# MeshFEM/MeshFEM

Measured on AMD Instinct MI355X. Metric: stiffness_assembly_elements_per_s, higher is better.
Workload: dtype f64; 1 GPU; configs[2]: 60^3 grid -> 5184000 P2 tets, isotropic E=200 nu=0.35, Dirichlet x=0, traction x=1; elements=5184000, nodes=7430761, dof=22292283, nnz_blocks=201443041, stored_blocks=104436901, matrix_storage=upper, parallelism=1 GPU, step=embed + Ke blocks + assembly into block-CSR (gather/owner-computes)

## Files before the change

meshfem_amd/csrc/mfh_api.cpp:

```cpp
#include "mfh_ctx.hh"
#include <dlfcn.h>

using namespace mfh;

namespace {
struct RoctxApi {
    int (*push)(const char *) = nullptr;
    int (*pop)() = nullptr;
    RoctxApi() {
        const char *en = getenv("MFH_ROCTX");
        if (!en || en[0] == '0') return;
        for (const char *lib : {"librocprofiler-sdk-roctx.so", "libroctx64.so", "/opt/rocm/lib/librocprofiler-sdk-roctx.so", "/opt/rocm/lib/libroctx64.so"}) {
            if (void *h = dlopen(lib, RTLD_NOW | RTLD_GLOBAL)) {
                push = reinterpret_cast<int (*)(const char *)>(dlsym(h, "roctxRangePushA"));
                pop = reinterpret_cast<int (*)()>(dlsym(h, "roctxRangePop"));
                if (push && pop) return;
                push = nullptr; pop = nullptr;
            }
        }
    }
};
RoctxApi &roctx_api() { static RoctxApi a; return a; }
}
mfh::RoctxRange::RoctxRange(const char *name) {
// ... 44 lines not shown
    c->neumannTraction.assign((size_t)m.nBE() * m.dim, 0.0);
    const size_t n = m.bdryNodes.size() * (size_t)m.dim;
    if (n > 0 && c->dirMask.size() == n && c->dirVal.size() == n) {
        parallel_assign(c->dirMask, n, (uint8_t)0);
        parallel_assign(c->dirVal, n, 0.0);
    } else {
        RawVec<uint8_t>().swap(c->dirMask);
        RawVec<double>().swap(c->dirVal);
    }
    c->deltaForces.clear();
}
void clear_fixed(mfh_ctx *c) {
    c->fixedVars.clear();
    c->fixedVals.clear();
    if (c->hFixedMask.size() == (size_t)c->bs() * c->nDoF) parallel_assign(c->hFixedMask, c->hFixedMask.size(), (uint8_t)0);
    else RawVec<uint8_t>().swap(c->hFixedMask);
    c->fixedUploaded = false;
    c->anyFixedNonzero = false;
    c->dinvValid = false;
    c->tl.valid = false;
    c->mg.valid = false;
}

void upload_mesh(mfh_ctx *c, bool deviceTables) {
    double t0 = now_ms();
    c->autoStretch = -1.0;
    if (!c->hostOnly && !deviceTables) {
        require_device(c);
        MFH_HIP(hipSetDevice(c->device));
        c->dElemNodes.upload(c->mesh.elemNodes, c->stream);
        c->dVertPos.upload(c->mesh.nodePos, c->stream);
    }
    c->timing.upload_ms = now_ms() - t0;
    c->haveMesh = true;
    c->external = false;
    c->geoValid = false;
    c->hGeoValid = false;
    c->dofForNode.clear();
    c->nDoF = c->mesh.nNode;
    build_shape_tables(c->mesh.dim, c->mesh.deg, c->tables);
    if (!c->hostOnly) { c->dPairTable.upload(c->tables.pairTable, c->stream); c->dMassTable.upload(c->tables.massRef, c->stream); }
    invalidate_symbolic(c);
    dist_detach(c);
    reset_bcs(c);
    clear_fixed(c);
}

void set_isotropic(mfh_ctx *c, double E, double nu) {
    double lam = (nu * E) / ((1.0 + nu) * (1.0 - 2.0 * nu));
    if (c->haveMesh && c->mesh.dim == 2) lam = (nu * E) / (1.0 - nu * nu);
    c->matMode = 0;
    c->matKind = MAT_ISO;
    c->matParams = {lam, E / (2.0 + 2.0 * nu), E, nu};
    c->geoValid = false;
    c->hGeoValid = false;
    invalidate_matrix(c);
}

void ensure_pass_events(mfh_ctx *c) {
    if (c->passEv[0]) return;
    for (auto &e : c->passEv) MFH_HIP(hipEventCreate(&e));
    MFH_HIP(hipHostMalloc((void **)&c->negHost, 2 * sizeof(int), hipHostMallocDefault));
}

void ensure_geometry(mfh_ctx *c, bool deferCheck) {
    require(c->haveMesh, MFH_ERR_STATE, "no mesh set");
    if (c->geoValid) return;
    require(!c->hostOnly, MFH_ERR_HIP, "host-only context (device -1): no HIP device, and there is no CPU fallback");
    require_device(c);
    MFH_HIP(hipSetDevice(c->device));
    const HostMesh &m = c->mesh;
    if (c->matParams.empty() && !c->dMatBorrowed) set_isotropic(c, 1.0, 0.3);
    if (c->matMode == 0 && !c->dMatBorrowed) {
        double E = c->matParams[2], nu = c->matParams[3];
        double lam = (nu * E) / ((1.0 + nu) * (1.0 - 2.0 * nu));
        if (m.dim == 2) lam = (nu * E) / (1.0 - nu * nu);
        c->matParams[0] = lam;
    }
    c->geoStride = c->matKind == MAT_ISO ? GEO_ISO_STRIDE : (c->matKind == MAT_ORTHO ? GEO_ORTHO_STRIDE : GEO_GEN_STRIDE);
    if (!c->dMatBorrowed) c->dMatParams.upload(c->matParams, c->stream);
    const double *dMat = c->dMatBorrowed ? c->dMatBorrowed : c->dMatParams.p;
    c->dGeo.alloc((size_t)m.nElem * c->geoStride);
    c->dNeg.alloc(2);
    c->dNeg.zero(c->stream);
    ensure_pass_events(c);
    MFH_HIP(hipEventRecord(c->passEv[0], c->stream));
    k::launch_geometry(m.dim, m.deg, c->matKind, m.nElem, c->dElemNodes.p, m.npe, c->dVertPos.p, dMat, c->matMode,
                       c->dGeo.p, c->geoStride, c->dNeg.p, c->stream);
    MFH_HIP(hipEventRecord(c->passEv[1], c->stream));
    MFH_HIP(hipMemcpyAsync(c->negHost, c->dNeg.p, 2 * sizeof(int), hipMemcpyDeviceToHost, c->stream));
    c->geoPending = true;
    if (!deferCheck) finish_geometry(c);
}

void finish_geometry(mfh_ctx *c) {
    if (!c->geoPending) return;
    c->geoPending = false;
    MFH_HIP(hipStreamSynchronize(c->stream));
    float ms = 0;
    MFH_HIP(hipEventElapsedTime(&ms, c->passEv[0], c->passEv[1]));
    c->timing.geometry_ms = ms;
    const int neg[2] = {c->negHost[0], c->negHost[1]};
    if (neg[0] > 0)
        throw Error(MFH_ERR_INVALID, "Mesh has negatively oriented elements.\nCorrect with: mesh_convert --reorientNegativeElements. (" +
                                         std::to_string(neg[0]) + " elements)");
    if (neg[1] > 0)
        throw Error(MFH_ERR_INVALID, std::string(c->matMode == 1 ? "Isotropic" : "Orthotropic") + " parameters of " + std::to_string(neg[1]) +
                                         " elements give an indefinite elasticity tensor (" +
                                         (c->matMode == 1 ? "need E > 0 and -1 < nu < 1/2, nu < 1 in plane stress" : "compliance matrix not positive definite") + ").");
    c->geoValid = true;
    c->hGeoValid = false;
}

const std::vector<double> &host_geo(mfh_ctx *c) {
    ensure_geometry(c);
    if (!c->hGeoValid) {
        c->hGeo.resize(c->dGeo.n);
        c->dGeo.download(c->hGeo.data(), c->dGeo.n, c->stream);
        c->hGeoValid = true;
    }
    return c->hGeo;
}

const int32_t *device_dof_map(mfh_ctx *c) {
    if (c->dofForNode.empty()) return nullptr;
    if (!c->dofUploaded) { c->dDofForNode.upload(c->dofForNode, c->stream); c->dofUploaded = true; }
    return c->dDofForNode.p;
}

void ensure_host_colidx(mfh_ctx *c) {
    if (!c->sym.colIdx.empty() || c->sym.nnzb == 0) return;
    c->sym.colIdx.resize((size_t)c->sym.nnzb);
    c->dColIdx.download(c->sym.colIdx.data(), c->sym.colIdx.size(), c->stream);
}

void refresh_storage_rule(mfh_ctx *c) {
    if (c->symValid && resolve_upper_storage(c) != c->upperOnly) { c->symValid = false; invalidate_matrix(c); }
}

void ensure_symbolic(mfh_ctx *c, bool wantScatter) {
    require(c->haveMesh, MFH_ERR_STATE, "no mesh set");
    refresh_storage_rule(c);
    if (c->symValid && (!wantScatter || c->symHasScatter)) return;
    c->upperOnly = resolve_upper_storage(c);
    RoctxRange range("Compress Matrix");
    double t0 = now_ms();
    if (!c->hostOnly && c->symbolicDevice && c->contribOrder == 1) {
        require_device(c);
        MFH_HIP(hipSetDevice(c->device));
        const bool directPacked = c->asmPackedCodes && !c->keepHostSymbolic;
// ... 27 lines not shown
        invalidate_matrix(c);
        return;
    }
    build_symbolic(c->mesh, c->dofForNode, c->nDoF, c->nOwnedDoF(), c->chunkSlots, c->contribOrder, wantScatter, c->sym, c->upperOnly);
    c->timing.symbolic_ms = now_ms() - t0;
    const Symbolic &S = c->sym;
    c->symHasScatter = wantScatter;
    if (c->hostOnly) { c->symValid = true; return; }
    MFH_HIP(hipSetDevice(c->device));
    c->dRowPtr.upload(S.rowPtr, c->stream);
    c->dColIdx.upload(S.colIdx, c->stream);
    c->dChunkRow.upload(S.chunkRow, c->stream);
    c->dSpmvChunkRow.upload(S.spmvChunkRow, c->stream);
    c->dContribPtr.upload(S.contribPtr, c->stream);
    c->dContribCode.upload(S.contribCode, c->stream);
    c->dContribSlot.upload(S.contribSlot, c->stream);
    if (wantScatter) c->dScatter.upload(S.scatterSlot, c->stream);
    pack_gather_codes(c);
    if (!c->keepHostSymbolic) {
        std::vector<uint32_t>().swap(c->sym.contribCode);
        std::vector<uint16_t>().swap(c->sym.contribSlot);
        std::vector<int32_t>().swap(c->sym.scatterSlot);
    }
    { mfh::PoolTag values(c->hierarchyLevel ? 0 : 1); c->dVals.alloc(tiled_count(S.nnzb, c->dim() * c->dim())); }
    c->symValid = true;
    ++c->listsGen;
    ++c->valsGen;
    invalidate_matrix(c);
}

void pack_gather_codes(mfh_ctx *c) {
    c->codesPacked = false;
    if (!c->asmPackedCodes || c->hostOnly || c->sym.nChunk() == 0) return;
    c->dChunkElemBase.alloc((size_t)c->sym.nChunk());
    DBuf<int> flag;
    flag.alloc(1);
    c->codesPacked = k::launch_pack_codes(c->sym.nChunk(), c->dContribPtr.p, c->dContribCode.p, c->mesh.npe, c->dChunkElemBase.p, flag.p, c->stream);
}

k::AsmArgs asm_args(mfh_ctx *c) {
    const HostMesh &m = c->mesh;
    k::AsmArgs a{};
    a.dim = m.dim; a.deg = m.deg; a.npe = m.npe; a.mat = c->asmMat();
    a.geoStride = c->geoStride; a.geo = c->dGeo.p; a.pairTable = c->dPairTable.p; a.massTable = c->dMassTable.p;
    for (int k2 = 0; k2 < 6; ++k2) a.pairConst[k2] = c->tables.pairConst[k2];
    a.nChunk = c->sym.nChunk(); a.chunkRow = c->dChunkRow.p; a.rowPtr = c->dRowPtr.p;
    a.contribPtr = c->dContribPtr.p; a.contribCode = c->dContribCode.p; a.contribSlot = c->dContribSlot.p;
    a.chunkSlots = c->sym.chunkSlots;
    a.nElem = m.nElem; a.scatterSlot = c->dScatter.p;
    a.vals = c->dVals.p; a.nnzb = c->sym.nnzb;
    a.xcd = c->xcdSwizzle;
    a.upperOnly = c->upperOnly ? 1 : 0;
    a.det = c->deterministic ? 1 : 0;
    a.chunkElemBase = c->codesPacked ? c->dChunkElemBase.p : nullptr;
    a.chunkOrder = nullptr;
    if (c->asmChunkOrder && !c->hostOnly && a.nChunk > 1 && c->symValid && c->dContribPtr.p && c->dContribCode.p && c->contribOrder == 1) {
        if (c->chunkOrderGen != c->listsGen) {
            DBuf<uint32_t> keys;
            keys.alloc((size_t)a.nChunk);
            k::launch_chunk_keys(a, keys.p, c->stream);
            std::vector<uint32_t> hk((size_t)a.nChunk);
            keys.download(hk.data(), hk.size(), c->stream);
            std::vector<int32_t> order((size_t)a.nChunk);
            for (int64_t b = 0; b < a.nChunk; ++b) order[(size_t)b] = (int32_t)b;
            std::stable_sort(order.begin(), order.end(), [&](int32_t x, int32_t y) { return hk[(size_t)x] < hk[(size_t)y]; });
            c->dChunkOrder.upload(order, c->stream);
            c->chunkOrderGen = c->listsGen;
        }
        a.chunkOrder = c->dChunkOrder.p;
    }
    return a;
}

void run_assembly(mfh_ctx *c, int mode) {
    c->dVals32.release();
    k::AsmArgs a = asm_args(c);
    if (mode == MFH_ASSEMBLE_ATOMIC) {
        c->dVals.zero(c->stream);
        k::launch_assemble_atomic(a, c->stream);
    } else {
        k::launch_assemble_gather(a, c->stream);
    }
}

void placement_trials(mfh_ctx *c) {
    c->placementGen = c->valsGen;
    c->placementMs.clear();
    c->placementNote.clear();
    const size_t n = c->dVals.n, bytes = n * sizeof(double);
    if (c->placementTrials <= 0 || c->hostOnly || c->external || bytes < ((size_t)256 << 20)) return;
    auto timed = [&]() {
        k::AsmArgs a = asm_args(c);
        double best = 1e300;
        for (int r = 0; r < 2; ++r) {
            EventTimer t(c->stream);
            k::launch_assemble_gather(a, c->stream);
            best = std::min(best, t.stop());
        }
        return best;
    };
    double best = timed();
    c->placementMs.push_back(best);
    std::vector<std::unique_ptr<DBuf<double>>> held;
    for (int trial = 0; trial < c->placementTrials; ++trial) {
        size_t fr = 0, tot = 0;
        if (hipMemGetInfo(&fr, &tot) != hipSuccess) { (void)hipGetLastError(); break; }
// ... 810 lines not shown
    std::copy(c->mesh.bdryParent.begin(), c->mesh.bdryParent.end(), out);
    return MFH_OK;
}
mfh_status mfh_mesh_get_boundary_elem_internal(const mfh_ctx *c, uint8_t *out) {
    if (!c || !c->haveMesh || !out) return MFH_ERR_STATE;
    std::copy(c->mesh.bdryInternal.begin(), c->mesh.bdryInternal.end(), out);
    return MFH_OK;
}
mfh_status mfh_mesh_get_boundary_nodes(const mfh_ctx *c, int32_t *out) {
    if (!c || !c->haveMesh || !out) return MFH_ERR_STATE;
    std::copy(c->mesh.bdryNodes.begin(), c->mesh.bdryNodes.end(), out);
    return MFH_OK;
}
mfh_status mfh_mesh_get_boundary_elem_geometry(const mfh_ctx *c, double *volume, double *normal) {
    if (!c || !c->haveMesh) return MFH_ERR_STATE;
    if (volume) std::copy(c->mesh.bdryVol.begin(), c->mesh.bdryVol.end(), volume);
    if (normal) std::copy(c->mesh.bdryNormal.begin(), c->mesh.bdryNormal.end(), normal);
    return MFH_OK;
}
mfh_status mfh_mesh_get_elem_volumes(mfh_ctx *c, double *out) {
    MFH_TRY(c)
    require(c && out, MFH_ERR_INVALID, "null argument");
    const std::vector<double> &g = host_geo(c);
    for (int64_t e = 0; e < c->mesh.nElem; ++e) out[e] = g[(size_t)e * c->geoStride + 12];
    MFH_CATCH(c)
}

mfh_status mfh_material_isotropic(mfh_ctx *c, double E, double nu) {
    MFH_TRY(c)
    require(c, MFH_ERR_INVALID, "null context");
    set_isotropic(c, E, nu);
    MFH_CATCH(c)
}

mfh_status mfh_material_const(mfh_ctx *c, const double *D) {
    MFH_TRY(c)
    require(c && D && c->haveMesh, MFH_ERR_STATE, "set the mesh before the material");
    const int d = c->dim(), fl = flat_len(d);
    c->matParams.clear();
    bool ortho = true;
    for (int r = 0; r < fl && ortho; ++r)
        for (int cc = r + 1; cc < fl; ++cc)
            if (cc >= d && D[r * fl + cc] != 0.0) { ortho = false; break; }
    if (ortho) {
        for (int r = 0; r < d; ++r)
            for (int cc = r; cc < d; ++cc) c->matParams.push_back(D[r * fl + cc]);
        for (int k2 = d; k2 < fl; ++k2) c->matParams.push_back(D[k2 * fl + k2]);
        c->matMode = 5; c->matKind = MAT_ORTHO;
    } else {
        for (int r = 0; r < fl; ++r)
            for (int cc = r; cc < fl; ++cc) c->matParams.push_back(D[r * fl + cc]);
        c->matMode = 2; c->matKind = MAT_GENERAL;
    }
    c->geoValid = false; c->hGeoValid = false;
    invalidate_matrix(c);
    MFH_CATCH(c)
}

mfh_status mfh_material_iso_field(mfh_ctx *c, const double *E, const double *nu) {
    MFH_TRY(c)
    require(c && E && nu && c->haveMesh, MFH_ERR_STATE, "set the mesh before the material");
    const int64_t n = c->mesh.nElem;
    c->matParams.assign((size_t)2 * n, 0.0);
    std::copy(E, E + n, c->matParams.begin());
    std::copy(nu, nu + n, c->matParams.begin() + n);
    c->matMode = 1; c->matKind = MAT_ISO;
    c->geoValid = false; c->hGeoValid = false;
    invalidate_matrix(c);
    MFH_CATCH(c)
}

mfh_status mfh_material_ortho_field(mfh_ctx *c, const double *params) {
    MFH_TRY(c)
    require(c && params && c->haveMesh, MFH_ERR_STATE, "set the mesh before the material");
    const int np = c->dim() == 3 ? 9 : 4;
    c->matParams.assign(params, params + (size_t)np * c->mesh.nElem);
    c->matMode = 3; c->matKind = MAT_ORTHO;
    c->geoValid = false; c->hGeoValid = false;
    invalidate_matrix(c);
    MFH_CATCH(c)
}

mfh_status mfh_material_tensor_field(mfh_ctx *c, const double *D) {
    MFH_TRY(c)
    require(c && D && c->haveMesh, MFH_ERR_STATE, "set the mesh before the material");
    const int fl = flat_len(c->dim());
    c->matParams.assign(D, D + (size_t)fl * fl * c->mesh.nElem);
    c->matMode = 4; c->matKind = MAT_GENERAL;
    c->geoValid = false; c->hGeoValid = false;
    invalidate_matrix(c);
    MFH_CATCH(c)
}

mfh_status mfh_material_get(mfh_ctx *c, int64_t elem, double *D) {
    MFH_TRY(c)
    require(c && D && c->haveMesh && elem >= 0 && elem < c->mesh.nElem, MFH_ERR_INVALID, "bad element");
    const std::vector<double> &g = host_geo(c);
    elem_D(c, &g[(size_t)elem * c->geoStride], D);
    MFH_CATCH(c)
}

mfh_status mfh_dof_map(mfh_ctx *c, const int32_t *dofForNode, int64_t nDoF) {
    MFH_TRY(c)
    require(c && c->haveMesh, MFH_ERR_STATE, "no mesh set");
    c->nOwnedDoFSet = -1;
    if (!dofForNode) {
        c->dofForNode.clear();
        c->nDoF = c->mesh.nNode;
        std::fill(c->mesh.bdryInternal.begin(), c->mesh.bdryInternal.end(), (uint8_t)0);
    } else {
        require(c->mesh.nOwned == c->mesh.nNode, MFH_ERR_UNSUPPORTED, "a DoF map on a partitioned mesh says which DoFs are this rank's rows: mfh_dof_map_partitioned");
        require(nDoF > 0 && nDoF <= c->mesh.nNode, MFH_ERR_INVALID, "bad nDoF");
        for (int64_t n = 0; n < c->mesh.nNode; ++n)
            require(dofForNode[n] >= 0 && dofForNode[n] < nDoF, MFH_ERR_INVALID, "DoF index out of range");
        c->dofForNode.assign(dofForNode, dofForNode + c->mesh.nNode);
        c->nDoF = nDoF;
    }
    invalidate_symbolic(c);
    clear_fixed(c);
    MFH_CATCH(c)
}

mfh_status mfh_dof_map_partitioned(mfh_ctx *c, const int32_t *dofForNode, int64_t nDoF, int64_t nOwnedDoF) {
    MFH_TRY(c)
    require(c && c->haveMesh && dofForNode, MFH_ERR_STATE, "no mesh set");
    require(!c->mesh.hasTopology, MFH_ERR_UNSUPPORTED, "partitioned contexts are built by mfh_mesh_set");
    require(nDoF > 0 && nDoF <= c->mesh.nNode && nOwnedDoF > 0 && nOwnedDoF <= nDoF, MFH_ERR_INVALID, "bad DoF counts");
    for (int64_t n = 0; n < c->mesh.nNode; ++n)
        require(dofForNode[n] >= 0 && dofForNode[n] < nDoF, MFH_ERR_INVALID, "DoF index out of range");
    c->dofForNode.assign(dofForNode, dofForNode + c->mesh.nNode);
    c->nDoF = nDoF;
    c->nOwnedDoFSet = nOwnedDoF;
    invalidate_symbolic(c);
    clear_fixed(c);
    dist_detach(c);
    MFH_CATCH(c)
}

mfh_status mfh_apply_periodic_conditions(mfh_ctx *c, double eps, int64_t *nDoF) {
    MFH_TRY(c)
    require(c && c->haveMesh, MFH_ERR_STATE, "no mesh set");
// ... 764 lines not shown
```

meshfem_amd/csrc/mfh_ctx.hh:

```
#pragma once
#include "mfh_internal.hh"
#include <cmath>
#include <map>
#include <mutex>

using namespace mfh;

struct mfh_ctx {
    int device = 0;
    bool hostOnly = false;
    bool hierarchyLevel = false;
    bool keepHostSymbolic = false;
    int xcdSwizzle = 0;
    RawVec<double> hLoad, hX, hXBatch, hLoadBatch;
    bool alwaysReembed = false;
    bool deterministic = false;
    DBuf<double> detPartials;
    DBuf<unsigned> detCounter;
    bool periodicIgnoreMismatch = false;
    int periodicIgnoreDims = 0;
    hipStream_t stream = nullptr;
    bool ownStream = true;
    bool arenaCounted = false;
    std::string err;

    HostMesh mesh;
    bool haveMesh = false;
    bool external = false;
    DBuf<int32_t> dElemNodes;
    DBuf<double> dVertPos;

    int matMode = 0;
    int matKind = MAT_ISO;
    int op = MFH_OP_ELASTICITY;
    std::vector<double> matParams;
    DBuf<double> dMatParams;
    const double *dMatBorrowed = nullptr;
    DBuf<double> dGeo;
    DBuf<int> dNeg;
    int geoStride = GEO_ISO_STRIDE;
    bool geoValid = false;
    hipEvent_t passEv[4] = {nullptr, nullptr, nullptr, nullptr};
    int *negHost = nullptr;
    bool geoPending = false;
    std::vector<double> hGeo;
    bool hGeoValid = false;

    std::vector<int32_t> dofForNode;
    DBuf<int32_t> dDofForNode;
    bool dofUploaded = false;
    int64_t nDoF = 0;

    Symbolic sym;
    bool symValid = false;
    bool symHasScatter = false;
    DBuf<int32_t> dRowPtr, dColIdx, dChunkRow, dSpmvChunkRow, dScatter;
    DBuf<int64_t> dContribPtr;
    int matrixStorage = -1;
    bool upperOnly = false;
    int nCU = 256;
    DBuf<uint32_t> dContribCode;
    DBuf<uint16_t> dContribSlot;
    ShapeTables tables;
    DBuf<double> dPairTable, dMassTable;
    MfLists mf;
    bool mfValid = false;
    int matrixFree = -1;
    bool use_mf() const {
        if (external || !haveMesh || hostOnly) return false;
        return matrixFree == 1 || (matrixFree < 0 && op == MFH_OP_ELASTICITY);
    }
    DBuf<int32_t> dMfChunkRow;
    DBuf<int64_t> dMfPairPtr;
    DBuf<uint32_t> dMfPairCode, dMfPairPos;
    DBuf<uint16_t> dMfPairRow;
    MfClusterLists mfc;
    MfClusterDev mfcDev;
    bool mfcValid = false;
    int mfXcdGroup = 32;
    bool mfReorder = true;
    DBuf<int32_t> dMfElemPerm, dMfElemNodes;
    int mfLaneStride = 37;
    bool mfGeoFromVerts = true;
    int mfBlockElems = 0;
    DBuf<double> dMfSig;
    int mfChunkRows = 256, mfChunkPairs = 2048;
    bool mfClusterUnfit = false;
    int mfModeEff() const { return (mfMode == 4 && mfClusterUnfit) ? 3 : mfMode; }
    int mfMode = 4;
// ... 304 lines not shown
```

meshfem_amd/csrc/mfh_internal.hh:

```
#pragma once
#include <hip/hip_runtime.h>
#include <cstdint>
#include <cstdio>
#include <cstring>
#include <string>
#include <vector>
#include <stdexcept>
#include <chrono>
#include <thread>
#include <functional>
#include <algorithm>
#include <array>
#include <memory>
#include <cstdlib>
#include "../../include/meshfem_hip.h"
#include "../../include/meshfem_hip_extras.h"

namespace mfh {

struct Error : std::runtime_error {
    mfh_status code;
    Error(mfh_status c, const std::string &m) : std::runtime_error(m), code(c) {}
};

// ... 267 lines not shown
void build_aggregates_device(int dim, int64_t nDoF, const double *dPos, int targetNodes, hipStream_t s, Aggregates &A,
                             DBuf<int32_t> &dAggOfDof, DBuf<double> &dRelPos, DBuf<int32_t> &dAggPtr, DBuf<int32_t> &dDofsByAgg,
                             const double *globalBox = nullptr, int64_t globalCount = 0, bool fullLattice = false, const double *aspect = nullptr);
void element_extent_sums_device(int dim, int64_t nElem, int npe, const int32_t *dElemNodes, const double *dPos, hipStream_t s, double out[3]);
void bounding_box_device(int dim, int64_t nDoF, const double *dPos, hipStream_t s, double mn[3], double mx[3]);
void wrap_positions_device(int64_t n, int dim, const double box[6], hipStream_t s, double *dPos, int skipDims = 0);
bool spd_inverse_inplace(int64_t n, double *A);
void build_mg_transfer_device(const HostMesh &m, const int32_t *dElemNodes, hipStream_t s, DBuf<int32_t> &parA, DBuf<int32_t> &parB,
                              DBuf<int32_t> &fineOf, DBuf<int32_t> &resPtr, DBuf<int32_t> &resIdx);

}

namespace mfh { namespace k {

struct DetBuf {
    double *partials = nullptr;
    unsigned *counter = nullptr;
    int cap = 0;
};
extern thread_local DetBuf t_det;
struct DetScope {
    DetBuf saved;
    explicit DetScope(const DetBuf &d) : saved(t_det) { t_det = d; }
    ~DetScope() { t_det = saved; }
    DetScope(const DetScope &) = delete;
    DetScope &operator=(const DetScope &) = delete;
};
inline int det_grid(int grid) { return t_det.partials ? std::min(grid, t_det.cap) : grid; }
void launch_det_finish(hipStream_t s);

struct AsmArgs {
    int dim, deg, npe, mat;
    int geoStride;
    const double *geo;
    const double *pairTable;
    const double *massTable;
    double pairConst[6];
    int64_t nChunk;
    const int32_t *chunkRow;
    const int32_t *rowPtr;
    const int64_t *contribPtr;
    const uint32_t *contribCode;
    const uint16_t *contribSlot;
    int chunkSlots;
    int64_t nElem;
    const int32_t *scatterSlot;
    double *vals;
    int64_t nnzb;
    int xcd;
    const int32_t *chunkElemBase;
    const int32_t *chunkOrder;
    int upperOnly;
    int det;
};

void launch_geometry(int dim, int deg, int mat, int64_t nElem, const int32_t *elemNodes, int npe,
                     const double *vertPos, const double *matParams, int matMode, double *geo, int geoStride,
                     int *negCount, hipStream_t s);
void launch_assemble_gather(const AsmArgs &a, hipStream_t s);
void launch_chunk_keys(const AsmArgs &a, uint32_t *keys, hipStream_t s);
bool launch_pack_codes(int64_t nChunk, const int64_t *contribPtr, uint32_t *contribCode, int npe, int32_t *chunkElemBase, int *flag, hipStream_t s);
void launch_assemble_atomic(const AsmArgs &a, hipStream_t s);
void launch_element_stiffness(const AsmArgs &a, int64_t first, int64_t count, double *KeOut, hipStream_t s);
void launch_constant_strain_load(const AsmArgs &a, const int32_t *elemNodes, const int32_t *dofForNode, const double *intGrad,
                                 const double *cstrain, const double *deltaP, double *out, hipStream_t s);
void launch_average_strain(const AsmArgs &a, const int32_t *elemNodes, const double *intGrad, const double *uNodes, double *out,
                           int wantStress, const double *uFixed, const double *deltaP, hipStream_t s, const double *addStrain = nullptr,
                           double *integral = nullptr);
void launch_apply_delta_K(const AsmArgs &a, const int32_t *elemNodes, const int32_t *dofForNode, const double *intGrad,
                          const double *uNodes, const double *deltaP, double *out, hipStream_t s);
void launch_mutual_energies(const AsmArgs &a, const int32_t *elemNodes, const double *intGrad, const double *w, int64_t nNode,
                            const double *deltaP, double *out, hipStream_t s);
void launch_boundary_strain_field(const AsmArgs &a, const int32_t *elemNodes, const double *intGrad, int64_t nBE,
                                  const int32_t *bdryParent, const int32_t *bdryElemNodes, int npbe, const double *uNodes,
                                  int wantStress, double *out, hipStream_t s);
void launch_strain_field(const AsmArgs &a, const int32_t *elemNodes, const double *intGrad, const double *uNodes, int wantStress,
                         double *out, hipStream_t s);
void launch_mutual_energy_differential(const AsmArgs &a, const int32_t *elemNodes, const double *intGrad, const double *w,
                                       int64_t nNode, int64_t nVert, double *out, hipStream_t s);
void launch_average_gradient(const AsmArgs &a, const int32_t *elemNodes, const double *intGrad, const double *uNodes, double *out,
                             hipStream_t s);

struct SpmvArgs {
    int dim;
    int64_t nChunk;
    const int32_t *chunkRow;
    const int32_t *rowPtr;
    const int32_t *colIdx;
    const double *vals;
    const float *vals32;
    int chunkSlots;
    const uint8_t *fixedMask;
    int xcd;
    int pcgMode;
    DetBuf det;
};
struct SpmvMfArgs {
    int dim, deg, npe, mat;
    int64_t nChunk;
    const int32_t *chunkRow;
    const int64_t *pairPtr;
    const uint32_t *pairCode;
    const uint16_t *pairRow;
    const uint32_t *pairPos;
    const int32_t *elemNodes;
    const int32_t *dofForNode;
// ... 154 lines not shown
```

meshfem_amd/csrc/mfh_kernels.hip:

```cpp
#include "mfh_device.hh"

namespace mfh { namespace k {

template <int DIM, int MAT> DEV constexpr int mat_nb() { return (MAT == MAT_LAPLACE || MAT == MAT_MASS) ? 1 : DIM * DIM; }

template <int DIM, int MAT>
DEV void block_from_H(const double *__restrict__ g, const double (&H)[DIM][DIM], double *K);

template <int DIM>
DEV void pair_H(const double *__restrict__ g, uint32_t offs , double S0, double S1, double S2,
                double S3, double (&H)[DIM][DIM]) {
#ifndef MFH_ASM_ABLATE
#define MFH_ASM_ABLATE 0
#endif
    const double vol = MFH_ASM_ABLATE >= 1 ? 1.0 : g[12];
    S0 *= vol; S1 *= vol; S2 *= vol; S3 *= vol;
    const char *gb = reinterpret_cast<const char *>(g);
    const double *gsi = reinterpret_cast<const double *>(gb + (offs & 0xffu)), *gti = reinterpret_cast<const double *>(gb + ((offs >> 8) & 0xffu)),
                 *gsj = reinterpret_cast<const double *>(gb + ((offs >> 16) & 0xffu)), *gtj = reinterpret_cast<const double *>(gb + (offs >> 24));
    double ua[DIM], ub[DIM], p[DIM], q[DIM];
#pragma unroll
    for (int a = 0; a < DIM; ++a) {
        ua[a] = MFH_ASM_ABLATE >= 1 ? S0 + a : gsi[a]; ub[a] = MFH_ASM_ABLATE >= 1 ? S1 - a : gti[a];
        const double va = MFH_ASM_ABLATE >= 2 ? S2 + a : gsj[a], vb = MFH_ASM_ABLATE >= 2 ? S3 - a : gtj[a];
        p[a] = S0 * va + S1 * vb;
        q[a] = S2 * va + S3 * vb;
    }
#pragma unroll
    for (int a = 0; a < DIM; ++a)
#pragma unroll
        for (int b = 0; b < DIM; ++b) H[a][b] = ua[a] * p[b] + ub[a] * q[b];
}

template <int DIM, int DEG, int MAT>
DEV void elem_block(const double *__restrict__ g, const double *__restrict__ pairTab, const PairConst &pc, int i, int j, double *K) {
    constexpr int NPE = (DIM == 3) ? (DEG == 1 ? 4 : 10) : (DEG == 1 ? 3 : 6);
    const double vol = g[12];
    if (MAT == MAT_MASS) {
        K[0] = vol * pairTab[i * NPE + j];
        return;
    }
    double H[DIM][DIM];
    if (DEG == 1) {
        double gi[DIM], gj[DIM];
#pragma unroll
        for (int a = 0; a < DIM; ++a) { gi[a] = g[i * DIM + a]; gj[a] = g[j * DIM + a] * vol; }
#pragma unroll
        for (int a = 0; a < DIM; ++a)
#pragma unroll
            for (int b = 0; b < DIM; ++b) H[a][b] = gi[a] * gj[b];
    } else {
        const int si = sup_s<DIM, DEG>(i), ti = sup_t<DIM, DEG>(i), sj = sup_s<DIM, DEG>(j), tj = sup_t<DIM, DEG>(j);
        constexpr int NV = DIM + 1;
        const bool vi = i < NV, vj = j < NV;
        const int lAi = vi ? si : ti, lBi = si, lAj = vj ? sj : tj, lBj = sj;
        const double c1 = pc.ee_ne, c2 = pc.ee_eq - pc.ee_ne, c3 = pc.ee_ne - pc.ve_ne;
        const double oi = vi ? 1.0 : 0.0, oj = vj ? 1.0 : 0.0;
        auto coef = [&](bool eq, double o, double o2) -> double { return (c1 + (eq ? c2 : 0.0)) - c3 * (o + o2) + o * o2; };
        double S0 = coef(lAi == lAj, oi, oj);
        double S1 = vj ? 0.0 : coef(lAi == lBj, oi, 0.0);
        double S2 = vi ? 0.0 : coef(lBi == lAj, 0.0, oj);
        double S3 = (vi | vj) ? 0.0 : coef(lBi == lBj, 0.0, 0.0);
        S0 *= vol; S1 *= vol; S2 *= vol; S3 *= vol;
        double ua[DIM], ub[DIM], p[DIM], q[DIM];
#pragma unroll
        for (int a = 0; a < DIM; ++a) {
            ua[a] = g[si * DIM + a]; ub[a] = g[ti * DIM + a];
            const double va = g[sj * DIM + a], vb = g[tj * DIM + a];
            p[a] = S0 * va + S1 * vb;
            q[a] = S2 * va + S3 * vb;
        }
#pragma unroll
        for (int a = 0; a < DIM; ++a)
#pragma unroll
            for (int b = 0; b < DIM; ++b) H[a][b] = ua[a] * p[b] + ub[a] * q[b];
    }
    block_from_H<DIM, MAT>(g, H, K);
}

template <int DIM, int MAT>
DEV void block_from_H(const double *__restrict__ g, const double (&H)[DIM][DIM], double *K) {
    if (MAT == MAT_LAPLACE) {
        double tr = 0;
#pragma unroll
        for (int a = 0; a < DIM; ++a) tr += H[a][a];
        K[0] = tr;
    } else if (MAT == MAT_ISO) {
#if defined(MFH_ASM_ABLATE) && MFH_ASM_ABLATE >= 1
        const double lam = H[0][0], mu = H[1][1];
#else
        const double lam = g[13], mu = g[14];
#endif
        double tr = 0;
#pragma unroll
        for (int a = 0; a < DIM; ++a) tr += H[a][a];
#pragma unroll
        for (int c = 0; c < DIM; ++c)
#pragma unroll
            for (int d = 0; d < DIM; ++d) K[c * DIM + d] = lam * H[c][d] + mu * H[d][c] + (c == d ? mu * tr : 0.0);
    } else if (MAT == MAT_ORTHO) {
#pragma unroll
        for (int c = 0; c < DIM; ++c)
#pragma unroll
            for (int d = 0; d < DIM; ++d) {
                double v = g[13 + npack<DIM>(c, d)] * H[c][d];
                if (c == d) {
#pragma unroll
                    for (int a = 0; a < DIM; ++a)
                        if (a != c) v += g[ortho_shear_offset<DIM>() + flat_idx<DIM>(a, c) - DIM] * H[a][a];
                } else v += g[ortho_shear_offset<DIM>() + flat_idx<DIM>(c, d) - DIM] * H[d][c];
                K[c * DIM + d] = v;
            }
    } else {
        constexpr int ND = (DIM * (DIM + 1) / 2) * (DIM * (DIM + 1) / 2 + 1) / 2;
        double D[ND];
#pragma unroll
        for (int k = 0; k < ND; ++k) D[k] = g[13 + k];
#pragma unroll
        for (int c = 0; c < DIM; ++c)
#pragma unroll
            for (int d = 0; d < DIM; ++d) {
                double acc = 0;
#pragma unroll
                for (int a = 0; a < DIM; ++a)
#pragma unroll
                    for (int b = 0; b < DIM; ++b) acc += H[a][b] * D[dpack<DIM>(flat_idx<DIM>(a, c), flat_idx<DIM>(d, b))];
                K[c * DIM + d] = acc;
            }
    }
}

template <int DIM>
DEV void embed_simplex(const double (&P)[DIM + 1][DIM], double (&gl)[DIM + 1][DIM], double &vol) {
    if (DIM == 3) {
        auto cross = [](const double *a, const double *b, double *o) {
            o[0] = a[1] * b[2] - a[2] * b[1]; o[1] = a[2] * b[0] - a[0] * b[2]; o[2] = a[0] * b[1] - a[1] * b[0];
        };
        double d31[3], d21[3], d01[3], d20[3], d30[3], d10[3], n[4][3];
#pragma unroll
        for (int a = 0; a < 3; ++a) {
            d31[a] = P[3][a] - P[1][a]; d21[a] = P[2][a] - P[1][a]; d01[a] = P[0][a] - P[1][a];
            d20[a] = P[2][a] - P[0][a]; d30[a] = P[3][a] - P[0][a]; d10[a] = P[1][a] - P[0][a];
        }
        cross(d31, d21, n[0]); cross(d20, d30, n[1]); cross(d30, d10, n[2]); cross(d10, d20, n[3]);
        const double vol6 = d01[0] * n[0][0] + d01[1] * n[0][1] + d01[2] * n[0][2];
        vol = vol6 / 6.0;
#pragma unroll
        for (int k = 0; k < 4; ++k)
#pragma unroll
            for (int a = 0; a < 3; ++a) gl[k][a] = n[k][a] / vol6;
    } else {
        double E[3][2];
// ... 63 lines not shown
            const double *q = mp + e * 4;
            const double a00 = 1.0 / q[0], a01 = -q[2] / q[1], a11 = 1.0 / q[1];
            const double det = a00 * a11 - a01 * a01;
            if (!(a00 > 0 && det > 0 && q[3] > 0)) atomicAdd(negCount + 1, 1);
            g[13 + npack<2>(0, 0)] = a11 / det; g[13 + npack<2>(0, 1)] = -a01 / det; g[13 + npack<2>(1, 1)] = a00 / det;
            g[ortho_shear_offset<2>()] = q[3];
        }
    } else {
        const double *q = mp + e * FL * FL;
        for (int r = 0; r < FL; ++r)
            for (int c = r; c < FL; ++c) g[13 + dpack<DIM>(r, c)] = q[r * FL + c];
    }
    }
    __syncthreads();
    const int64_t e0 = (int64_t)blockIdx.x * blockDim.x;
    const int nLive = (int)(nElem - e0 < (int64_t)blockDim.x ? nElem - e0 : (int64_t)blockDim.x);
    double *out = geo + e0 * stride;
    for (int q = threadIdx.x; q < nLive * stride; q += blockDim.x) {
        const int el = q / stride;
        out[q] = recs[(size_t)el * (stride + 1) + (q - el * stride)];
    }
}

template <int DIM, int DEG, int MAT> DEV constexpr bool asm_uses_table() { return DEG == 2 && MAT != MAT_MASS; }
constexpr int ASM_CODE_SHIFT = 7;

template <int DIM, int DEG, int MAT, bool UPPER = false, bool DET = false>
__global__ void __launch_bounds__(256, (MAT == MAT_GENERAL || MAT == MAT_ORTHO) ? 1 : 8) k_assemble_gather(AsmArgs a) {
    constexpr int NB = mat_nb<DIM, MAT>();
    constexpr int NPE = (DIM == 3) ? (DEG == 1 ? 4 : 10) : (DEG == 1 ? 3 : 6);
    constexpr bool TAB = asm_uses_table<DIM, DEG, MAT>();
    extern __shared__ __attribute__((aligned(16))) double acc[];
    const int CS = a.chunkSlots + 2;
    double *tabS = acc + (size_t)NB * CS;
    uint32_t *tabO = reinterpret_cast<uint32_t *>(tabS + NPE * NPE * 4);
    uint32_t *turn = tabO + NPE * NPE;
    const PairConst pc{a.pairConst[0], a.pairConst[1], a.pairConst[2], a.pairConst[3], a.pairConst[4], a.pairConst[5]};
    const int64_t item = a.xcd == 1 ? xcd_item(blockIdx.x, gridDim.x) : (a.xcd > 1 ? xcd_group_item(blockIdx.x, gridDim.x, a.xcd) : (int64_t)blockIdx.x);
    const int64_t chunk = a.chunkOrder ? (int64_t)a.chunkOrder[item] : item;
    const int r0 = a.chunkRow[chunk], r1 = a.chunkRow[chunk + 1];
    const int s0 = a.rowPtr[r0];
    const int ns = a.rowPtr[r1] - s0;
    const uint32_t eBase = a.chunkElemBase ? (uint32_t)a.chunkElemBase[chunk] : 0u;
    const int par = s0 & 1;
    for (int t = threadIdx.x; t < ns + par; t += 256)
#pragma unroll
        for (int c = 0; c < NB; ++c) acc[c * CS + t] = 0.0;
    if (DET && threadIdx.x == 0) *turn = 0u;
    if (TAB) {
        for (int t = threadIdx.x; t < NPE * NPE; t += 256) {
            const int i = t / NPE, j = t - i * NPE;
#pragma unroll
            for (int k = 0; k < 4; ++k) tabS[t * 4 + k] = a.pairTable[t * 4 + k];
            tabO[t] = (uint32_t)(sup_s<DIM, DEG>(i) * DIM * 8) | ((uint32_t)(sup_t<DIM, DEG>(i) * DIM * 8) << 8) |
                      ((uint32_t)(sup_s<DIM, DEG>(j) * DIM * 8) << 16) | ((uint32_t)(sup_t<DIM, DEG>(j) * DIM * 8) << 24);
        }
    }
    __syncthreads();
    const int64_t kb = a.contribPtr[chunk], ke = a.contribPtr[chunk + 1];
    constexpr int U = 2;
    constexpr bool det = DET;
    unsigned turnNo = threadIdx.x >> 6;
    for (int64_t k0 = kb + threadIdx.x; det ? (k0 - threadIdx.x < ke) : (k0 < ke); k0 += 256 * U) {
        uint32_t code[U];
        int ls[U];
        bool ok[U];
#pragma unroll
        for (int u = 0; u < U; ++u) {
            const int64_t kk = k0 + (int64_t)u * 256;
            ok[u] = kk < ke;
            code[u] = ok[u] ? a.contribCode[kk] : a.contribCode[kb];
            ls[u] = (ok[u] ? (int)a.contribSlot[kk] : 0) + par;
        }
#pragma unroll
        for (int u = 0; u < U; ++u) {
            double K[NB];
            if (ok[u]) {
            uint32_t e;
            int ij;
            if (a.chunkElemBase) { e = eBase + (code[u] >> ASM_CODE_SHIFT); ij = (int)(code[u] & ((1u << ASM_CODE_SHIFT) - 1)); }
            else { e = code[u] / (NPE * NPE); ij = (int)(code[u] - e * (NPE * NPE)); }
            const double *g = a.geo + (int64_t)e * a.geoStride;
            if (TAB) {
                typedef double dv2 __attribute__((ext_vector_type(2)));
                const dv2 s01 = *reinterpret_cast<const dv2 *>(&tabS[ij * 4]), s23 = *reinterpret_cast<const dv2 *>(&tabS[ij * 4 + 2]);
                const uint32_t offs = tabO[ij];
                double H[DIM][DIM];
                pair_H<DIM>(g, offs, s01.x, s01.y, s23.x, s23.y, H);
                block_from_H<DIM, MAT>(g, H, K);
            } else {
                const int i = ij / NPE, j = ij - i * NPE;
                elem_block<DIM, DEG, MAT>(g, MAT == MAT_MASS ? a.massTable : a.pairTable, pc, i, j, K);
            }
            }
            if (det) {
                if ((threadIdx.x & 63) == 0)
                    while (__hip_atomic_load(turn, __ATOMIC_ACQUIRE, __HIP_MEMORY_SCOPE_WORKGROUP) != turnNo) __builtin_amdgcn_s_sleep(1);
                if (ok[u]) {
#pragma unroll
                    for (int c = 0; c < NB; ++c) unsafeAtomicAdd(&acc[c * CS + ls[u]], K[c]);
                }
                __builtin_amdgcn_fence(__ATOMIC_RELEASE, "workgroup");
                if ((threadIdx.x & 63) == 0) __hip_atomic_store(turn, turnNo + 1u, __ATOMIC_RELEASE, __HIP_MEMORY_SCOPE_WORKGROUP);
                turnNo += 4u;
            } else if (ok[u]) {
#pragma unroll
                for (int c = 0; c < NB; ++c) unsafeAtomicAdd(&acc[c * CS + ls[u]], K[c]);
            }
            __builtin_amdgcn_sched_barrier(0);
        }
    }
    __syncthreads();
    const int nl = ns + par;
    const int64_t sbase = (int64_t)s0 - par;
    const int pfirst = par;
    const int plast = nl >> 1;
    for (int p = pfirst + threadIdx.x; p < plast; p += 256) {
        const int t = 2 * p;
        const int64_t s = sbase + t;
#pragma unroll
        for (int c = 0; c < NB; ++c) {
            const double2 v = *reinterpret_cast<const double2 *>(&acc[c * CS + t]);
            double2 *dst = reinterpret_cast<double2 *>(&a.vals[tiled_index(s, c, NB)]);
            typedef double dv2 __attribute__((ext_vector_type(2)));
            dv2 w = {v.x, v.y};
            __builtin_nontemporal_store(w, reinterpret_cast<dv2 *>(dst));
        }
    }
    if (threadIdx.x < 2) {
        const int t = threadIdx.x == 0 ? 1 : nl - 1;
        const bool live = threadIdx.x == 0 ? (par == 1 && nl > 1) : ((nl & 1) && nl - 1 >= par && !(par == 1 && nl - 1 == 1));
        if (live) {
            const int64_t s = sbase + t;
#pragma unroll
            for (int c = 0; c < NB; ++c) a.vals[tiled_index(s, c, NB)] = acc[c * CS + t];
        }
    }
}

__global__ void __launch_bounds__(256) k_chunk_keys(int64_t nChunk, const int64_t *__restrict__ contribPtr, const uint32_t *__restrict__ contribCode,
                                                    const int32_t *__restrict__ chunkElemBase, uint32_t npe2, uint32_t *__restrict__ keys) {
    const int64_t b = (int64_t)blockIdx.x * 256 + threadIdx.x;
    if (b >= nChunk) return;
    const int64_t kb = contribPtr[b], ke = contribPtr[b + 1];
    if (ke <= kb) { keys[b] = 0xffffffffu; return; }
    const uint32_t c = contribCode[kb + (ke - kb) / 2];
    keys[b] = chunkElemBase ? (uint32_t)chunkElemBase[b] + (c >> ASM_CODE_SHIFT) : c / npe2;
}

__global__ void __launch_bounds__(64) k_pack_codes(int64_t nChunk, const int64_t *__restrict__ contribPtr, uint32_t *__restrict__ contribCode,
                                                   uint32_t npe2, int32_t *__restrict__ chunkElemBase, int *flag, int rewrite) {
    const int64_t b = blockIdx.x;
    const int64_t kb = contribPtr[b], ke = contribPtr[b + 1];
    if (rewrite) {
        const uint32_t lo = (uint32_t)chunkElemBase[b];
        for (int64_t k = kb + threadIdx.x; k < ke; k += 64) {
            const uint32_t c = contribCode[k], e = c / npe2;
            contribCode[k] = ((e - lo) << ASM_CODE_SHIFT) | (c - e * npe2);
        }
        return;
    }
    uint32_t lo = 0xffffffffu, hi = 0;
    for (int64_t k = kb + threadIdx.x; k < ke; k += 64) {
        const uint32_t e = contribCode[k] / npe2;
// ... 1538 lines not shown
}


void launch_geometry(int dim, int , int , int64_t nElem, const int32_t *elemNodes, int npe, const double *vertPos,
                     const double *matParams, int matMode, double *geo, int geoStride, int *negCount, hipStream_t s) {
    const int grid = (int)((nElem + 255) / 256);
    const size_t lds = (size_t)256 * (geoStride + 1) * sizeof(double);
    if (lds > 64 * 1024) {
        MFH_HIP(hipFuncSetAttribute((const void *)k_geometry<3>, hipFuncAttributeMaxDynamicSharedMemorySize, (int)lds));
        MFH_HIP(hipFuncSetAttribute((const void *)k_geometry<2>, hipFuncAttributeMaxDynamicSharedMemorySize, (int)lds));
    }
    if (dim == 3) hipLaunchKernelGGL(k_geometry<3>, dim3(grid), dim3(256), lds, s, nElem, elemNodes, npe, vertPos, matParams, matMode, geo, geoStride, negCount);
    else hipLaunchKernelGGL(k_geometry<2>, dim3(grid), dim3(256), lds, s, nElem, elemNodes, npe, vertPos, matParams, matMode, geo, geoStride, negCount);
    CHECK_LAUNCH();
}

#define MFH_DISPATCH(a, CALL)                                                            \
    do {                                                                                 \
        const int key_ = (a.dim == 3 ? 0 : 6) + (a.deg == 2 ? 3 : 0) + (a.mat == MAT_GENERAL ? 1 : (a.mat == MAT_ORTHO ? 2 : 0)); \
        switch (key_) {                                                                  \
        case 0: { CALL(3, 1, MAT_ISO); } break;                                           \
        case 1: { CALL(3, 1, MAT_GENERAL); } break;                                       \
        case 2: { CALL(3, 1, MAT_ORTHO); } break;                                         \
        case 3: { CALL(3, 2, MAT_ISO); } break;                                           \
        case 4: { CALL(3, 2, MAT_GENERAL); } break;                                       \
        case 5: { CALL(3, 2, MAT_ORTHO); } break;                                         \
        case 6: { CALL(2, 1, MAT_ISO); } break;                                           \
        case 7: { CALL(2, 1, MAT_GENERAL); } break;                                       \
        case 8: { CALL(2, 1, MAT_ORTHO); } break;                                         \
        case 9: { CALL(2, 2, MAT_ISO); } break;                                           \
        case 10: { CALL(2, 2, MAT_GENERAL); } break;                                      \
        default: { CALL(2, 2, MAT_ORTHO); } break;                                        \
        }                                                                                \
    } while (0)

#define MFH_DISPATCH_ASM(a, CALL)                                                        \
    do {                                                                                 \
        if (!mat_is_scalar(a.mat)) { MFH_DISPATCH(a, CALL); break; }                     \
        const int key_ = (a.dim == 3 ? 0 : 4) + (a.deg == 2 ? 2 : 0) + (a.mat == MAT_MASS ? 1 : 0); \
        switch (key_) {                                                                  \
        case 0: { CALL(3, 1, MAT_LAPLACE); } break;                                       \
        case 1: { CALL(3, 1, MAT_MASS); } break;                                          \
        case 2: { CALL(3, 2, MAT_LAPLACE); } break;                                       \
        case 3: { CALL(3, 2, MAT_MASS); } break;                                          \
        case 4: { CALL(2, 1, MAT_LAPLACE); } break;                                       \
        case 5: { CALL(2, 1, MAT_MASS); } break;                                          \
        case 6: { CALL(2, 2, MAT_LAPLACE); } break;                                       \
        default: { CALL(2, 2, MAT_MASS); } break;                                         \
        }                                                                                \
    } while (0)

void launch_assemble_gather(const AsmArgs &a, hipStream_t s) {
    if (a.nChunk == 0) return;
    size_t lds = (size_t)(mat_is_scalar(a.mat) ? 1 : a.dim * a.dim) * (a.chunkSlots + 2) * sizeof(double);
    if (a.deg == 2 && a.mat != MAT_MASS) lds += (size_t)a.npe * a.npe * (4 * sizeof(double) + sizeof(uint32_t));
    if (a.det) lds = (size_t)(mat_is_scalar(a.mat) ? 1 : a.dim * a.dim) * (a.chunkSlots + 2) * sizeof(double) + (size_t)a.npe * a.npe * (4 * sizeof(double) + sizeof(uint32_t)) + 16;
#define CALLV(D, G, M, UP, DT)                                                                                 \
    do {                                                                                                         \
        if (lds > 64 * 1024)                                                                                     \
            MFH_HIP(hipFuncSetAttribute((const void *)k_assemble_gather<D, G, M, UP, DT>, hipFuncAttributeMaxDynamicSharedMemorySize, (int)lds)); \
        hipLaunchKernelGGL((k_assemble_gather<D, G, M, UP, DT>), dim3((unsigned)a.nChunk), dim3(256), lds, s, a); \
    } while (0)
#define CALL(D, G, M)                                                     \
    if (a.det) { if (a.upperOnly) CALLV(D, G, M, true, true); else CALLV(D, G, M, false, true); } \
    else { if (a.upperOnly) CALLV(D, G, M, true, false); else CALLV(D, G, M, false, false); }
    MFH_DISPATCH_ASM(a, CALL);
#undef CALL
#undef CALLV
    CHECK_LAUNCH();
}

void launch_chunk_keys(const AsmArgs &a, uint32_t *keys, hipStream_t s) {
    if (a.nChunk == 0) return;
    hipLaunchKernelGGL(k_chunk_keys, dim3((unsigned)((a.nChunk + 255) / 256)), dim3(256), 0, s, a.nChunk, a.contribPtr, a.contribCode,
                       a.chunkElemBase, (uint32_t)(a.npe * a.npe), keys);
    CHECK_LAUNCH();
}

bool launch_pack_codes(int64_t nChunk, const int64_t *contribPtr, uint32_t *contribCode, int npe, int32_t *chunkElemBase, int *flag, hipStream_t s) {
    if (nChunk == 0) return true;
    MFH_HIP(hipMemsetAsync(flag, 0, sizeof(int), s));
    hipLaunchKernelGGL(k_pack_codes, dim3((unsigned)nChunk), dim3(64), 0, s, nChunk, contribPtr, contribCode, (uint32_t)(npe * npe), chunkElemBase, flag, 0);
    CHECK_LAUNCH();
    int h = 0;
    MFH_HIP(hipMemcpyAsync(&h, flag, sizeof(int), hipMemcpyDeviceToHost, s));
    MFH_HIP(hipStreamSynchronize(s));
    if (h) return false;
    hipLaunchKernelGGL(k_pack_codes, dim3((unsigned)nChunk), dim3(64), 0, s, nChunk, contribPtr, contribCode, (uint32_t)(npe * npe), chunkElemBase, flag, 1);
    CHECK_LAUNCH();
    return true;
}

void launch_assemble_atomic(const AsmArgs &a, hipStream_t s) {
    const int64_t total = a.nElem * a.npe * a.npe;
    const int grid = grid_for(total, 256 * 32);
#define CALL(D, G, M) hipLaunchKernelGGL((k_assemble_atomic<D, G, M>), dim3(grid), dim3(256), 0, s, a)
    MFH_DISPATCH_ASM(a, CALL);
#undef CALL
    CHECK_LAUNCH();
}

void launch_element_stiffness(const AsmArgs &a, int64_t first, int64_t count, double *KeOut, hipStream_t s) {
    const int grid = grid_for(count * a.npe * a.npe);
#define CALL(D, G, M) hipLaunchKernelGGL((k_element_stiffness<D, G, M>), dim3(grid), dim3(256), 0, s, a, first, count, KeOut)
    MFH_DISPATCH_ASM(a, CALL);
#undef CALL
// ... 344 lines not shown
```

Measured before the change: 1.660 billion elements/s.

## Pass constant isotropic Lamé parameters as kernel args and vectorize gradient loads

When the material is a single isotropic constant, the assembly kernel now takes lambda and mu as kernel arguments instead of reading them from each element's geometry record. The per-pair gradient fetch changes from byte-offset pointer loads to 16-byte vector loads of the whole gradient block followed by register selects. The neg-orientation device-to-host copy moves into finish_geometry, and material parameters are re-uploaded only when they change. These changes reduce per-contribution memory traffic and address arithmetic, at the cost of extra selects, more registers, and a new alignment requirement on element records.

```diff
diff --git a/meshfem_amd/csrc/mfh_api.cpp b/meshfem_amd/csrc/mfh_api.cpp
--- a/meshfem_amd/csrc/mfh_api.cpp
+++ b/meshfem_amd/csrc/mfh_api.cpp
@@ -120,6 +120,7 @@
     c->matMode = 0;
     c->matKind = MAT_ISO;
     c->matParams = {lam, E / (2.0 + 2.0 * nu), E, nu};
+    c->matDirty = true;
     c->geoValid = false;
     c->hGeoValid = false;
     invalidate_matrix(c);
@@ -143,10 +144,10 @@
         double E = c->matParams[2], nu = c->matParams[3];
         double lam = (nu * E) / ((1.0 + nu) * (1.0 - 2.0 * nu));
         if (m.dim == 2) lam = (nu * E) / (1.0 - nu * nu);
-        c->matParams[0] = lam;
+        if (c->matParams[0] != lam) { c->matParams[0] = lam; c->matDirty = true; }
     }
     c->geoStride = c->matKind == MAT_ISO ? GEO_ISO_STRIDE : (c->matKind == MAT_ORTHO ? GEO_ORTHO_STRIDE : GEO_GEN_STRIDE);
-    if (!c->dMatBorrowed) c->dMatParams.upload(c->matParams, c->stream);
+    if (!c->dMatBorrowed && (c->matDirty || !c->dMatParams.p)) { c->dMatParams.upload(c->matParams, c->stream); c->matDirty = false; }
     const double *dMat = c->dMatBorrowed ? c->dMatBorrowed : c->dMatParams.p;
     c->dGeo.alloc((size_t)m.nElem * c->geoStride);
     c->dNeg.alloc(2);
@@ -156,7 +157,6 @@
     k::launch_geometry(m.dim, m.deg, c->matKind, m.nElem, c->dElemNodes.p, m.npe, c->dVertPos.p, dMat, c->matMode,
                        c->dGeo.p, c->geoStride, c->dNeg.p, c->stream);
     MFH_HIP(hipEventRecord(c->passEv[1], c->stream));
-    MFH_HIP(hipMemcpyAsync(c->negHost, c->dNeg.p, 2 * sizeof(int), hipMemcpyDeviceToHost, c->stream));
     c->geoPending = true;
     if (!deferCheck) finish_geometry(c);
 }
@@ -164,6 +164,7 @@
 void finish_geometry(mfh_ctx *c) {
     if (!c->geoPending) return;
     c->geoPending = false;
+    MFH_HIP(hipMemcpyAsync(c->negHost, c->dNeg.p, 2 * sizeof(int), hipMemcpyDeviceToHost, c->stream));
     MFH_HIP(hipStreamSynchronize(c->stream));
     float ms = 0;
     MFH_HIP(hipEventElapsedTime(&ms, c->passEv[0], c->passEv[1]));
@@ -297,6 +298,8 @@
     a.xcd = c->xcdSwizzle;
     a.upperOnly = c->upperOnly ? 1 : 0;
     a.det = c->deterministic ? 1 : 0;
+    a.constMat = (c->matMode == 0 && !c->dMatBorrowed && c->matParams.size() >= 2) ? 1 : 0;
+    if (a.constMat) { a.lam = c->matParams[0]; a.mu = c->matParams[1]; }
     a.chunkElemBase = c->codesPacked ? c->dChunkElemBase.p : nullptr;
     a.chunkOrder = nullptr;
     if (c->asmChunkOrder && !c->hostOnly && a.nChunk > 1 && c->symValid && c->dContribPtr.p && c->dContribCode.p && c->contribOrder == 1) {
@@ -1213,6 +1216,7 @@
             for (int cc = r; cc < fl; ++cc) c->matParams.push_back(D[r * fl + cc]);
         c->matMode = 2; c->matKind = MAT_GENERAL;
     }
+    c->matDirty = true;
     c->geoValid = false; c->hGeoValid = false;
     invalidate_matrix(c);
     MFH_CATCH(c)
@@ -1226,6 +1230,7 @@
     std::copy(E, E + n, c->matParams.begin());
     std::copy(nu, nu + n, c->matParams.begin() + n);
     c->matMode = 1; c->matKind = MAT_ISO;
+    c->matDirty = true;
     c->geoValid = false; c->hGeoValid = false;
     invalidate_matrix(c);
     MFH_CATCH(c)
@@ -1237,6 +1242,7 @@
     const int np = c->dim() == 3 ? 9 : 4;
     c->matParams.assign(params, params + (size_t)np * c->mesh.nElem);
     c->matMode = 3; c->matKind = MAT_ORTHO;
+    c->matDirty = true;
     c->geoValid = false; c->hGeoValid = false;
     invalidate_matrix(c);
     MFH_CATCH(c)
@@ -1248,6 +1254,7 @@
     const int fl = flat_len(c->dim());
     c->matParams.assign(D, D + (size_t)fl * fl * c->mesh.nElem);
     c->matMode = 4; c->matKind = MAT_GENERAL;
+    c->matDirty = true;
     c->geoValid = false; c->hGeoValid = false;
     invalidate_matrix(c);
     MFH_CATCH(c)
diff --git a/meshfem_amd/csrc/mfh_ctx.hh b/meshfem_amd/csrc/mfh_ctx.hh
--- a/meshfem_amd/csrc/mfh_ctx.hh
+++ b/meshfem_amd/csrc/mfh_ctx.hh
@@ -35,6 +35,7 @@
     int op = MFH_OP_ELASTICITY;
     std::vector<double> matParams;
     DBuf<double> dMatParams;
+    bool matDirty = true;
     const double *dMatBorrowed = nullptr;
     DBuf<double> dGeo;
     DBuf<int> dNeg;
diff --git a/meshfem_amd/csrc/mfh_internal.hh b/meshfem_amd/csrc/mfh_internal.hh
--- a/meshfem_amd/csrc/mfh_internal.hh
+++ b/meshfem_amd/csrc/mfh_internal.hh
@@ -343,6 +343,8 @@
     const int32_t *chunkOrder;
     int upperOnly;
     int det;
+    int constMat;
+    double lam, mu;
 };
 
 void launch_geometry(int dim, int deg, int mat, int64_t nElem, const int32_t *elemNodes, int npe,
diff --git a/meshfem_amd/csrc/mfh_kernels.hip b/meshfem_amd/csrc/mfh_kernels.hip
--- a/meshfem_amd/csrc/mfh_kernels.hip
+++ b/meshfem_amd/csrc/mfh_kernels.hip
@@ -8,28 +8,55 @@
 DEV void block_from_H(const double *__restrict__ g, const double (&H)[DIM][DIM], double *K);
 
 template <int DIM>
-DEV void pair_H(const double *__restrict__ g, uint32_t offs , double S0, double S1, double S2,
-                double S3, double (&H)[DIM][DIM]) {
+DEV void iso_block(double lam, double mu, const double (&H)[DIM][DIM], double *K) {
+    double tr = 0;
+#pragma unroll
+    for (int a = 0; a < DIM; ++a) tr += H[a][a];
+#pragma unroll
+    for (int c = 0; c < DIM; ++c)
+#pragma unroll
+        for (int d = 0; d < DIM; ++d) K[c * DIM + d] = lam * H[c][d] + mu * H[d][c] + (c == d ? mu * tr : 0.0);
+}
+
+DEV double sel2(bool b, double x0, double x1) { double r = x0; if (b) r = x1; return r; }
+
+template <int DIM>
+DEV void pair_H(const double *__restrict__ g, uint32_t sel , double vol, double S0, double S1,
+                double S2, double S3, double (&H)[DIM][DIM]) {
 #ifndef MFH_ASM_ABLATE
 #define MFH_ASM_ABLATE 0
 #endif
-    const double vol = MFH_ASM_ABLATE >= 1 ? 1.0 : g[12];
+    typedef double dv2 __attribute__((ext_vector_type(2)));
+    const dv2 *gv = reinterpret_cast<const dv2 *>(g);
+    const dv2 abl = {S0, S1};
+    const dv2 r0 = MFH_ASM_ABLATE >= 2 ? abl : gv[0], r1 = MFH_ASM_ABLATE >= 2 ? abl : gv[1], r2 = MFH_ASM_ABLATE >= 2 ? abl : gv[2];
+    dv2 r3 = abl, r4 = abl, r5 = abl;
+    if (DIM == 3 && MFH_ASM_ABLATE < 2) { r3 = gv[3]; r4 = gv[4]; r5 = gv[5]; }
+    auto grad = [&](int a, bool b0, bool b1) -> double {
+        if (DIM == 3) {
+            if (a == 0) return sel2(b1, sel2(b0, r0.x, r1.y), sel2(b0, r3.x, r4.y));
+            if (a == 1) return sel2(b1, sel2(b0, r0.y, r2.x), sel2(b0, r3.y, r5.x));
+            return sel2(b1, sel2(b0, r1.x, r2.y), sel2(b0, r4.x, r5.y));
+        }
+        if (a == 0) return sel2(b1, sel2(b0, r0.x, r1.x), r2.x);
+        return sel2(b1, sel2(b0, r0.y, r1.y), r2.y);
+    };
     S0 *= vol; S1 *= vol; S2 *= vol; S3 *= vol;
-    const char *gb = reinterpret_cast<const char *>(g);
-    const double *gsi = reinterpret_cast<const double *>(gb + (offs & 0xffu)), *gti = reinterpret_cast<const double *>(gb + ((offs >> 8) & 0xffu)),
-                 *gsj = reinterpret_cast<const double *>(gb + ((offs >> 16) & 0xffu)), *gtj = reinterpret_cast<const double *>(gb + (offs >> 24));
-    double ua[DIM], ub[DIM], p[DIM], q[DIM];
+    const bool si0 = sel & 1u, si1 = sel & 2u, ti0 = sel & 4u, ti1 = sel & 8u, sj0 = sel & 16u, sj1 = sel & 32u, tj0 = sel & 64u, tj1 = sel & 128u;
+    double p[DIM], q[DIM];
 #pragma unroll
     for (int a = 0; a < DIM; ++a) {
-        ua[a] = MFH_ASM_ABLATE >= 1 ? S0 + a : gsi[a]; ub[a] = MFH_ASM_ABLATE >= 1 ? S1 - a : gti[a];
-        const double va = MFH_ASM_ABLATE >= 2 ? S2 + a : gsj[a], vb = MFH_ASM_ABLATE >= 2 ? S3 - a : gtj[a];
+        const double va = grad(a, sj0, sj1), vb = grad(a, tj0, tj1);
         p[a] = S0 * va + S1 * vb;
         q[a] = S2 * va + S3 * vb;
     }
-#pragma unroll
-    for (int a = 0; a < DIM; ++a)
-#pragma unroll
-        for (int b = 0; b < DIM; ++b) H[a][b] = ua[a] * p[b] + ub[a] * q[b];
+    __builtin_amdgcn_sched_barrier(0);
+#pragma unroll
+    for (int a = 0; a < DIM; ++a) {
+        const double ua = grad(a, si0, si1), ub = grad(a, ti0, ti1);
+#pragma unroll
+        for (int b = 0; b < DIM; ++b) H[a][b] = ua * p[b] + ub * q[b];
+    }
 }
 
 template <int DIM, int DEG, int MAT>
@@ -86,18 +113,7 @@
         for (int a = 0; a < DIM; ++a) tr += H[a][a];
         K[0] = tr;
     } else if (MAT == MAT_ISO) {
-#if defined(MFH_ASM_ABLATE) && MFH_ASM_ABLATE >= 1
-        const double lam = H[0][0], mu = H[1][1];
-#else
-        const double lam = g[13], mu = g[14];
-#endif
-        double tr = 0;
-#pragma unroll
-        for (int a = 0; a < DIM; ++a) tr += H[a][a];
-#pragma unroll
-        for (int c = 0; c < DIM; ++c)
-#pragma unroll
-            for (int d = 0; d < DIM; ++d) K[c * DIM + d] = lam * H[c][d] + mu * H[d][c] + (c == d ? mu * tr : 0.0);
+        iso_block<DIM>(g[13], g[14], H, K);
     } else if (MAT == MAT_ORTHO) {
 #pragma unroll
         for (int c = 0; c < DIM; ++c)
@@ -267,25 +283,30 @@
             const int i = t / NPE, j = t - i * NPE;
 #pragma unroll
             for (int k = 0; k < 4; ++k) tabS[t * 4 + k] = a.pairTable[t * 4 + k];
-            tabO[t] = (uint32_t)(sup_s<DIM, DEG>(i) * DIM * 8) | ((uint32_t)(sup_t<DIM, DEG>(i) * DIM * 8) << 8) |
-                      ((uint32_t)(sup_s<DIM, DEG>(j) * DIM * 8) << 16) | ((uint32_t)(sup_t<DIM, DEG>(j) * DIM * 8) << 24);
+            tabO[t] = (uint32_t)sup_s<DIM, DEG>(i) | ((uint32_t)sup_t<DIM, DEG>(i) << 2) | ((uint32_t)sup_s<DIM, DEG>(j) << 4) |
+                      ((uint32_t)sup_t<DIM, DEG>(j) << 6);
         }
     }
     __syncthreads();
     const int64_t kb = a.contribPtr[chunk], ke = a.contribPtr[chunk + 1];
+    const uint32_t *__restrict__ codes = a.contribCode + kb;
+    const uint16_t *__restrict__ slots = a.contribSlot + kb;
+    const uint32_t nk = (uint32_t)(ke - kb);
     constexpr int U = 2;
     constexpr bool det = DET;
     unsigned turnNo = threadIdx.x >> 6;
-    for (int64_t k0 = kb + threadIdx.x; det ? (k0 - threadIdx.x < ke) : (k0 < ke); k0 += 256 * U) {
+    auto contributions = [&](auto constMat) {
+    constexpr bool CM = decltype(constMat)::value;
+    for (uint32_t k0 = threadIdx.x; det ? (k0 - threadIdx.x < nk) : (k0 < nk); k0 += 256 * U) {
         uint32_t code[U];
         int ls[U];
         bool ok[U];
 #pragma unroll
         for (int u = 0; u < U; ++u) {
-            const int64_t kk = k0 + (int64_t)u * 256;
-            ok[u] = kk < ke;
-            code[u] = ok[u] ? a.contribCode[kk] : a.contribCode[kb];
-            ls[u] = (ok[u] ? (int)a.contribSlot[kk] : 0) + par;
+            const uint32_t kk = k0 + (uint32_t)u * 256;
+            ok[u] = kk < nk;
+            code[u] = ok[u] ? codes[kk] : codes[0];
+            ls[u] = (ok[u] ? (int)slots[kk] : 0) + par;
         }
 #pragma unroll
         for (int u = 0; u < U; ++u) {
@@ -299,10 +320,22 @@
             if (TAB) {
                 typedef double dv2 __attribute__((ext_vector_type(2)));
                 const dv2 s01 = *reinterpret_cast<const dv2 *>(&tabS[ij * 4]), s23 = *reinterpret_cast<const dv2 *>(&tabS[ij * 4 + 2]);
-                const uint32_t offs = tabO[ij];
+                const uint32_t sel = tabO[ij];
                 double H[DIM][DIM];
-                pair_H<DIM>(g, offs, s01.x, s01.y, s23.x, s23.y, H);
-                block_from_H<DIM, MAT>(g, H, K);
+                if (MAT == MAT_ISO) {
+                    double vol, lam = a.lam, mu = a.mu;
+                    if (MFH_ASM_ABLATE >= 1) { vol = 1.0; lam = s01.x; mu = s01.y; }
+                    else if (CM) vol = g[12];
+                    else {
+                        const dv2 vl = *reinterpret_cast<const dv2 *>(g + 12), m = *reinterpret_cast<const dv2 *>(g + 14);
+                        vol = vl.x; lam = vl.y; mu = m.x;
+                    }
+                    pair_H<DIM>(g, sel, vol, s01.x, s01.y, s23.x, s23.y, H);
+                    iso_block<DIM>(lam, mu, H, K);
+                } else {
+                    pair_H<DIM>(g, sel, MFH_ASM_ABLATE >= 1 ? 1.0 : g[12], s01.x, s01.y, s23.x, s23.y, H);
+                    block_from_H<DIM, MAT>(g, H, K);
+                }
             } else {
                 const int i = ij / NPE, j = ij - i * NPE;
                 elem_block<DIM, DEG, MAT>(g, MAT == MAT_MASS ? a.massTable : a.pairTable, pc, i, j, K);
@@ -325,6 +358,9 @@
             __builtin_amdgcn_sched_barrier(0);
         }
     }
+    };
+    if (TAB && MAT == MAT_ISO && a.constMat) contributions(std::true_type());
+    else contributions(std::false_type());
     __syncthreads();
     const int nl = ns + par;
     const int64_t sbase = (int64_t)s0 - par;
@@ -1969,6 +2005,8 @@
 
 void launch_assemble_gather(const AsmArgs &a, hipStream_t s) {
     if (a.nChunk == 0) return;
+    if ((reinterpret_cast<uintptr_t>(a.geo) & 15u) != 0 || (a.geoStride & 1) != 0)
+        throw mfh::Error(MFH_ERR_STATE, "element records are not 16-byte aligned");
     size_t lds = (size_t)(mat_is_scalar(a.mat) ? 1 : a.dim * a.dim) * (a.chunkSlots + 2) * sizeof(double);
     if (a.deg == 2 && a.mat != MAT_MASS) lds += (size_t)a.npe * a.npe * (4 * sizeof(double) + sizeof(uint32_t));
     if (a.det) lds = (size_t)(mat_is_scalar(a.mat) ? 1 : a.dim * a.dim) * (a.chunkSlots + 2) * sizeof(double) + (size_t)a.npe * a.npe * (4 * sizeof(double) + sizeof(uint32_t)) + 16;
```

Result: faster. 1.727 billion elements/s, median of 6 (+4.0%).
